# ryought/dbgphmm

Hardware: AMD Instinct MI355X
Metric: read-bases/sec through forward+backward P(R|X) (higher is better)
Workload: dtype f64; 1 GPU; cfg3: synthetic 100 kb diploid genome (1% divergence), 20x HiFi reads (p=0.001, L=1000), k=40 DBG; sparse-adaptive forward+backward+posteriors (generate_mappings); n_nodes=131694, n_edges=132357, reads_rank0=4026, bases_rank0=4000713, total_bases=4000713, spin_up_steps=12

## Files before the change

dbgphmm_amd/csrc/api.cpp:

```cpp
#include <chrono>
#include <cstdlib>
#include <cmath>
#include <cstring>

#include "phmm_internal.h"

namespace phmm {

static thread_local std::string g_error;
static thread_local hipStream_t g_stream = nullptr;
static thread_local uint64_t g_ws_limit = 0;
static thread_local CallStats g_stats;
static thread_local bool g_timing = false;

void set_error(const std::string &msg) { g_error = msg; }
int fail(int code, const std::string &msg) {
    g_error = msg;
    return code;
}
hipStream_t current_stream() { return g_stream; }
int &workset_index() {
    static thread_local int idx = 0;
    return idx;
}
// ... 50 lines not shown
    if (k.wide_bwd_t != 128 && k.wide_bwd_t != 448) k.wide_bwd_t = 0;
    k.wide_hinted_cpb = num("PHMM_WIDE_HINTED_CPB", 0);
    if (k.wide_hinted_cpb != 1 && k.wide_hinted_cpb != 2 && k.wide_hinted_cpb != 4) k.wide_hinted_cpb = 0;
    k.no_side_worker = flag("PHMM_NO_SIDE_WORKER");
    k.no_wide_handover = flag("PHMM_NO_WIDE_HANDOVER");
    k.workers = std::max(1, std::min(MAX_WORKERS, num("PHMM_WORKERS", 1)));
    k.warm_cols = num("PHMM_WARM_COLS", 0);
    k.chunk_groups = std::max(0, num("PHMM_CHUNK_GROUPS", 0));
    k.no_keep_all = flag("PHMM_NO_KEEP_ALL");
    k.pipeline_min_groups = std::max(1, num("PHMM_PIPELINE_MIN_GROUPS", 8));
    k.no_runmax = flag("PHMM_NO_RUNMAX");
    k.force_radix = flag("PHMM_FORCE_RADIX");
    k.no_bwd_skip = flag("PHMM_NO_BWD_SKIP");
    k.serial_emit = flag("PHMM_SERIAL_EMIT");
    k.emit_high_priority = flag("PHMM_EMIT_HIGH_PRIORITY");
    k.no_dma = flag("PHMM_NO_DMA");
    k.bwd_dma = flag("PHMM_BWD_DMA");
    k.dense_streams = num("PHMM_DENSE_STREAMS", 0);
    k.dense_w = num("PHMM_DENSE_W", 0);
    k.dense_npt = num("PHMM_DENSE_NPT", 0);
    if (const char *e = std::getenv("PHMM_MEM_FRACTION")) k.mem_fraction = std::min(0.97, std::max(0.1, std::atof(e)));
    k.share_prefix = num("PHMM_SHARE_PREFIX", -1);
    if (k.share_prefix < 0 || k.share_prefix > 6) k.share_prefix = -1;
    g_knobs = k;
}

void trace(const char *tag) {
    if (!g_knobs.trace) return;
    static thread_local std::chrono::steady_clock::time_point last = std::chrono::steady_clock::now();
    (void)hipStreamSynchronize(g_stream);
    const auto now = std::chrono::steady_clock::now();
    static const auto t0 = std::chrono::steady_clock::now();
    std::fprintf(stderr, "[phmm trace] w%d @%9.2f %-28s %8.2f ms\n", workset_index(),
                 std::chrono::duration<double, std::milli>(now - t0).count(), tag,
                 std::chrono::duration<double, std::milli>(now - last).count());
    last = now;
}

uint64_t table_budget(const DevicePool &pool, uint64_t reserve) {
    if (g_ws_limit) return g_ws_limit;
    size_t fr = 0, tot = 0;
    if (hipMemGetInfo(&fr, &tot) != hipSuccess) return (uint64_t)16 << 30;
    const double frac = g_knobs.mem_fraction > 0.0 ? g_knobs.mem_fraction : 0.9;
    const double b = frac * (double)(fr + pool.owned_table_bytes()) - (double)reserve;
    return (uint64_t)std::max(b, 64.0 * 1024 * 1024);
}
// ... 60 lines not shown
}
void flush_spare_buffers() { device_pool().flush_spares(); }

void DevicePool::release() {
    flush_spares();
    for (auto &w : wsets) w.release();
    ws_out.release();
    for (auto &ws : wstream)
        if (ws) {
            (void)hipStreamDestroy(ws);
            ws = nullptr;
        }
    for (auto &ws : cstream)
        if (ws) {
            (void)hipStreamDestroy(ws);
            ws = nullptr;
        }
    for (auto &we : cevent)
        for (auto &e : we)
            if (e) {
                (void)hipEventDestroy(e);
                e = nullptr;
            }
}

void copy_out(void *dst, const void *src_dev, size_t bytes) {
    if (!dst || !bytes) return;
    hipPointerAttribute_t at;
    const bool dev = hipPointerGetAttributes(&at, dst) == hipSuccess && at.type == hipMemoryTypeDevice;
    if (!dev) (void)hipGetLastError();
    HIP_CHECK(hipMemcpyAsync(dst, src_dev, bytes, dev ? hipMemcpyDeviceToDevice : hipMemcpyDeviceToHost,
                             current_stream()));
    HIP_CHECK(hipStreamSynchronize(current_stream()));
}

void put_bytes(void *dst, const void *src, size_t n) {
    if (!dst || !n) return;
    hipPointerAttribute_t at;
    if (hipPointerGetAttributes(&at, dst) == hipSuccess && at.type == hipMemoryTypeDevice) {
        HIP_CHECK(hipMemcpyAsync(dst, src, n, hipMemcpyHostToDevice, current_stream()));
        HIP_CHECK(hipStreamSynchronize(current_stream()));
    } else {
        (void)hipGetLastError();
        std::memcpy(dst, src, n);
    }
}
// ... 867 lines not shown
```

dbgphmm_amd/csrc/dense.hip:

```cpp
#include <algorithm>
#include <cmath>
#include <cstring>
#include <numeric>
#include <type_traits>

#include "dense_internal.h"
#include "lds_dma.h"
#include "prefix_share.h"

#ifndef PHMM_FWD_PF
#define PHMM_FWD_PF 2
#endif
#ifndef PHMM_BWD_PF
#define PHMM_BWD_PF 1
#endif
#ifndef PHMM_SMALLW_WAVES
#define PHMM_SMALLW_WAVES 3
#endif

namespace phmm {


__device__ __forceinline__ int xcd_block(int b, int nblk8) {
    int per = nblk8 >> 3;
// ... 66 lines not shown
        v += ror(v, std::integral_constant<int, 0x128>());
        v += ror(v, std::integral_constant<int, 0x124>());
        v += ror(v, std::integral_constant<int, 0x122>());
        v += ror(v, std::integral_constant<int, 0x121>());
        return v;
    }
#pragma unroll
    for (int off = 1; off < W; off <<= 1) v += __shfl_xor(v, off);
    return v;
}

struct OpMax {
    __device__ double operator()(double a, double b) const { return a > b ? a : b; }
};
struct OpAdd {
    __device__ double operator()(double a, double b) const { return a + b; }
};

template <int W, bool DMA>
__global__ void __launch_bounds__(BLOCK, (W == 64 ? 4 : PHMM_SMALLW_WAVES)) fwd_step(const DenseArgs a, const int pos) {
    __shared__ double lds[(BLOCK / 64) * 64];
    constexpr bool DMA_ = DMA && W == 64;
    __shared__ double ring[DMA_ ? (BLOCK / 64) * DMA_DEPTH * 128 : 1];
    const int g = blockIdx.y + a.g_off;
    const int lb = xcd_block(blockIdx.x, a.nblk8);
    constexpr int ROWS = BLOCK / W;
    const int r = threadIdx.x % W;
    const int row = threadIdx.x / W;
    const int len = a.len[g * W + r];
    const bool active = a.wf_sw == nullptr || a.wf_sw[g * W + r] < 0;
    const bool newcol = active && pos < len;
    const bool have_prev = active && pos >= 1 && pos <= len;
    const bool fin = have_prev && pos == len;
    if (!__syncthreads_or(newcol || have_prev)) return;
    const LinParams &lp = a.lp;
    const size_t NW = (size_t)a.N * W;

    int Epos = 0;
    double sc = 1.0, isc = 1.0, ibs = 0.0;
    double thrL = INFINITY, thrU = INFINITY;
    bool collect = false;
    if (have_prev) {
        const unsigned long long cm = a.cmaxF[((size_t)g * a.Lc + (pos - 1)) * W + r];
        const int Eprev = a.FE[((size_t)g * (a.Lc + 1) + (pos - 1)) * W + r];
        const double ib_st = exp(a.logib[pos - 1] - (double)Eprev * LN2);
        const unsigned long long ibb = (unsigned long long)__double_as_longlong(ib_st);
// ... 1397 lines not shown
```

dbgphmm_amd/csrc/dense_internal.h:

```cpp
#pragma once

#include <vector>

#include "phmm_internal.h"
#include "seg_hull.h"

namespace phmm {

static constexpr double LN2 = 0.693147180559945309417232121458;
static constexpr int BLOCK = 256;

struct DenseArgs {
    int N, ng, Lc, nblk, npt;
    int g_off;
    const NodeRec *nodes;
    const uint8_t *emis;
    const double *init, *dinit, *tdinit;
    const uint32_t *fc_off;
    const FwdEntry *fc;
    const uint32_t *bc_off;
    const BwdEntry *bc;
    const uint32_t *fh_off, *bh_off;
    const HopEntry *fh, *bh;
    int hop_mode;
    LinParams lp;
    const double *logib;
    const uint8_t *bases;
// ... 8 lines not shown
    double *Bm, *Bi, *Bd;
    int bcols;
    int *BE;
    unsigned long long *cmaxB;
    double *bpart;
    double *logmbB, *logibB;
    double *accg;
    int want_freq;
    int nblk8;
    unsigned long long *tmaxF;
    const int *bstart;
    int want_map;
    double *Pa, *Pb;
    double *Prun;
    unsigned long long *pmax;
    const int *wf_sw;
    const uint8_t *wf_mode;
    int *wf_sub;
    int *wf_cnt;
    uint32_t *wf_node;
    double *wf_tot;
    double wf_ratio;
    double wf_ub_a, wf_ub_b;
    const uint32_t *rs_off = nullptr, *rs = nullptr;
    uint32_t *skH = nullptr;
    uint8_t *skA = nullptr;
    int nrun = 0, nseg = 0, sseg = 1;
    unsigned long long *skcells = nullptr;
    const double *vFm = nullptr, *vFi = nullptr, *vFd = nullptr;
    const uint32_t *vlane = nullptr;
    int vLc = 0, vJ = 0;
};
static constexpr int WF_CAP = 1024;


struct Plan {
    int W, ng_total, npt, nblk, nblk8;
    std::vector<uint32_t> order;
};

Plan make_plan(const phmm_model *m, const phmm_reads *reads, int forced_w);
Plan make_plan_ids(const phmm_model *m, const phmm_reads *reads, const std::vector<uint32_t> &ids);
void layout(DenseArgs &a, int W, bool full_b, void *tables, void *misc, size_t &tb, size_t &mb,
            bool backward_only = false);
void fill_model_args(DenseArgs &a, const phmm_model *m);
void host_logib(const phmm_model *m, size_t n, std::vector<double> &out);
// ... 17 lines not shown
```

dbgphmm_amd/csrc/mapping_flow.hip:

```cpp
#include <algorithm>
#include <cmath>
#include <cstring>
#include <memory>

#include <hipcub/hipcub.hpp>

#include "sparse_dyn.h"
#include "lean_bwd_kernel.h"
#include "wide_bwd_kernel.h"

namespace phmm {

static constexpr int KMAX = PHMM_MAX_ACTIVE_NODES;

template <int CAP> struct FRec {
    double m[CAP], i[CAP], d[CAP];
    uint32_t id[CAP];
    int n, na, E;
};

template <int CAP> __device__ bool load_record(const RecPool &p, uint64_t pos_index, FRec<CAP> &f) {
    const uint64_t o1 = p.off[pos_index];
    if (o1 == 0) return false;
    const uint8_t *rec = p.base + (o1 - 8);
// ... 1151 lines not shown
                hipLaunchKernelGGL(emit_dense_small, dim3((unsigned)std::min(1024, (ub + BLOCK / 64 - 1) / (BLOCK / 64))), dim3(BLOCK), 0,
                                   s2, ma, pos, lanes);
                hipLaunchKernelGGL(emit_dense_map, dim3((unsigned)ub), dim3(BLOCK), 0, s2, ma, pos, lanes);
            }
            HIP_CHECK(hipEventRecord(ev_emit[par], s2));
            emitted[par] = true;
            if (st_on) st.launches[1]++;
        }
        for (int par = 0; par < 2; par++)
            if (emitted[par]) HIP_CHECK(hipStreamWaitEvent(s, ev_emit[par], 0));
        HIP_CHECK(hipGetLastError());
        const bool want_lb = mc.logb_out && pos_max >= 0 && lanes > 0;
        if (want_lb) {
            launch_bwd_finish(W, a);
            hipLaunchKernelGGL(gather_logb, dim3((unsigned)((lanes + BLOCK - 1) / BLOCK)), dim3(BLOCK), 0, s, (const double *)a.logmbB,
                               a.Lc, W, lanes, (double *)(cp + o_lb));
            HIP_CHECK(hipGetLastError());
        }
        st.ms[1] += lt.total_ms();
        for (int gi = 0; gi < lanes; gi++)
            if (st_on && !a.skcells && hb[gi] >= 0) st.cells[1] += (uint64_t)((hb[gi] & ~(1 << 30)) + 1) * m->N;
        const size_t err_words = (o_cells + sizeof(unsigned long long) - o_err) / sizeof(uint32_t);
        std::vector<uint32_t> herr(err_words);
        HIP_CHECK(hipMemcpyAsync(herr.data(), cp + o_err, sizeof(uint32_t) * err_words, hipMemcpyDeviceToHost, s));
        if (want_lb) HIP_CHECK(hipMemcpyAsync(mc.logb_out, cp + o_lb, sizeof(double) * lanes, hipMemcpyDeviceToHost, s));
        HIP_CHECK(hipStreamSynchronize(s));
        if (a.skcells) {
            unsigned long long nc = 0;
            memcpy(&nc, herr.data() + (o_cells - o_err) / sizeof(uint32_t), sizeof nc);
            st.cells[1] += nc;
        }
        if (dense_lock.owns_lock()) dense_lock.unlock();
        trace("  dense backward+collect");
        bool pool_full = false;
        for (int gi = 0; gi < lanes; gi++) {
            if (herr[gi] & SP_ERR_POOL) pool_full = true;
            else if (herr[gi] & ~SP_STOP_SLICE) PHMM_THROW(PHMM_EINTERNAL, "mapping backward error " + std::to_string(herr[gi]));
        }
        if (!pool_full) break;
        (void)attempt;
        throw SinkOverflow{};
    }
}

__global__ void __launch_bounds__(BLOCK) map_counts(RecPool mp, uint64_t n_pos, uint64_t *cnt) {
    const uint64_t p = (uint64_t)blockIdx.x * BLOCK + threadIdx.x;
    if (p > n_pos) return;
    uint64_t c = 0;
    if (p < n_pos) {
// ... 91 lines not shown
static void finish_mappings(phmm_model *m, const phmm_reads *reads, MappingSink &sink, const std::vector<double> &lf,
                            const std::vector<double> &lb, phmm_mappings **out, double *out_node_freq) {
    hipStream_t s = current_stream();
    const uint64_t n_pos = reads->total;
    std::unique_ptr<phmm_mappings> mp(new phmm_mappings());
    mp->R = reads->R;
    mp->total_pos = n_pos;
    mp->read_off = reads->off;
    mp->read_logp = lf;
    mp->read_logp_backward = lb;
    mp->host_valid = false;
    mp->trusted = true;
    (void)hipGetDevice(&mp->device);
    DevicePool &dpool = device_pool();
    DevBuf &cnt = m->wset().aux[13], &tmp = m->wset().aux[14];
    cnt.reserve(sizeof(uint64_t) * (n_pos + 1));
    dpool.take(mp->d_pos_off, sizeof(uint64_t) * (n_pos + 1));
    const unsigned nb = (unsigned)((n_pos + 1 + BLOCK - 1) / BLOCK);
    hipLaunchKernelGGL(map_counts, dim3(nb), dim3(BLOCK), 0, s, sink.mp, n_pos, cnt.as<uint64_t>());
    size_t tb = 0;
    HIP_CHECK(hipcub::DeviceScan::ExclusiveSum(nullptr, tb, cnt.as<uint64_t>(), mp->d_pos_off.as<uint64_t>(), (int)(n_pos + 1), s));
    tmp.reserve(tb);
    HIP_CHECK(hipcub::DeviceScan::ExclusiveSum(tmp.p, tb, cnt.as<uint64_t>(), mp->d_pos_off.as<uint64_t>(), (int)(n_pos + 1), s));
    uint64_t total = 0;
    HIP_CHECK(hipMemcpyAsync(&total, mp->d_pos_off.as<uint64_t>() + n_pos, sizeof(uint64_t), hipMemcpyDeviceToHost, s));
    HIP_CHECK(hipStreamSynchronize(s));
    mp->total_entries = total;
    dpool.take(mp->d_nodes, sizeof(uint32_t) * std::max<uint64_t>(total, 1));
    dpool.take(mp->d_logp, sizeof(double) * std::max<uint64_t>(total, 1));
    hipLaunchKernelGGL(map_compact, dim3(nb), dim3(BLOCK), 0, s, sink.mp, n_pos, mp->d_pos_off.as<uint64_t>(),
                       mp->d_nodes.as<uint32_t>(), mp->d_logp.as<double>());
    DevBuf &d_roff = m->wset().aux[15], &d_rmax = m->wset().aux[16];
    d_roff.upload(reads->off.data(), sizeof(uint64_t) * (reads->R + 1));
    d_rmax.reserve(sizeof(uint32_t) * reads->R);
    hipLaunchKernelGGL(map_read_max, dim3((unsigned)((reads->R + BLOCK / 64 - 1) / (BLOCK / 64))), dim3(BLOCK), 0, s,
                       d_roff.as<uint64_t>(), reads->R, mp->d_pos_off.as<uint64_t>(), d_rmax.as<uint32_t>());
    mp->read_max_list.resize(reads->R);
    HIP_CHECK(hipMemcpyAsync(mp->read_max_list.data(), d_rmax.p, sizeof(uint32_t) * reads->R, hipMemcpyDeviceToHost, s));
    HIP_CHECK(hipStreamSynchronize(s));
    mp->on_device = true;
    trace("device CSR");
    if (out_node_freq) {
        DevBuf &d_prob = m->wset().aux[17], &d_sn = m->wset().aux[18], &d_sp = m->wset().aux[19], &d_freq = m->wset().aux[20];
        const uint64_t n = std::max<uint64_t>(total, 1);
        d_prob.reserve(sizeof(double) * n);
        d_sn.reserve(sizeof(uint32_t) * n);
        d_sp.reserve(sizeof(double) * n);
        d_freq.reserve(sizeof(double) * m->N);
        if (total) {
            hipLaunchKernelGGL(map_probs, dim3((unsigned)((total + BLOCK - 1) / BLOCK)), dim3(BLOCK), 0, s,
                               mp->d_logp.as<double>(), total, d_prob.as<double>());
            int end_bit = 1;
            while (end_bit < 32 && (1ull << end_bit) < m->N) end_bit++;
            size_t sb = 0;
            HIP_CHECK(hipcub::DeviceRadixSort::SortPairs(nullptr, sb, mp->d_nodes.as<uint32_t>(), d_sn.as<uint32_t>(),
                                                         d_prob.as<double>(), d_sp.as<double>(), (int)total, 0, end_bit, s));
            tmp.reserve(sb);
            HIP_CHECK(hipcub::DeviceRadixSort::SortPairs(tmp.p, sb, mp->d_nodes.as<uint32_t>(), d_sn.as<uint32_t>(),
                                                         d_prob.as<double>(), d_sp.as<double>(), (int)total, 0, end_bit, s));
        }
        hipLaunchKernelGGL(map_node_freq, dim3((m->N + NODE_FREQ_WAVES - 1) / NODE_FREQ_WAVES), dim3(64 * NODE_FREQ_WAVES), 0, s, d_sn.as<uint32_t>(),
// ... 659 lines not shown
```

dbgphmm_amd/csrc/phmm_internal.h:

```cpp
#pragma once

#include <hip/hip_runtime.h>

#include <cstdint>
#include <cstdio>
#include <memory>
#include <mutex>
#include <string>
#include <vector>

#include "../../include/phmm_amd.h"
#include "../../include/phmm_amd_states.h"
#include "../../include/phmm_amd_path.h"
#include "../../include/phmm_amd_share.h"
#include "../../include/phmm_amd_sample.h"
#include "../../include/phmm_amd_generate.h"
#include "../../include/phmm_amd_align.h"

namespace phmm {

void set_error(const std::string &msg);
int fail(int code, const std::string &msg);

struct Error {
    int code;
    std::string msg;
};
#define PHMM_THROW(code, msg) throw ::phmm::Error{(code), (msg)}
// ... 63 lines not shown
void copy_out(void *dst, const void *src_dev, size_t bytes);

struct WorkSet {
    DevBuf tables, misc, aux[24];
    size_t bytes() const {
        size_t b = tables.bytes + misc.bytes;
        for (const auto &a : aux) b += a.bytes;
        return b;
    }
    void release() {
        tables.release();
        misc.release();
        for (auto &a : aux) a.release();
    }
};
static constexpr int MAX_WORKERS = 4;
struct DevicePool {
    int device = 0;
    std::recursive_mutex call_mu;
    WorkSet wsets[MAX_WORKERS];
    hipStream_t wstream[MAX_WORKERS] = {};
    hipStream_t cstream[MAX_WORKERS] = {};
    hipEvent_t cevent[MAX_WORKERS][4] = {};
    DevBuf ws_out;
    static constexpr size_t SPARE_MAX = 6, SPARE_BYTES = (size_t)8 << 30;
    std::mutex spare_mu;
    std::vector<std::pair<void *, size_t>> spare;
    size_t spare_total = 0;
    void recycle(DevBuf &b);
    void take(DevBuf &b, size_t n);
    void flush_spares();
    size_t owned_table_bytes() const {
        size_t b = 0;
        for (const auto &w : wsets) b += w.tables.bytes;
        return b;
    }
    size_t owned_bytes() const {
        size_t b = ws_out.bytes + spare_total;
        for (const auto &w : wsets) b += w.bytes();
        return b;
    }
    void release();
};
DevicePool &device_pool();

struct LinParams {
    double p_mismatch, p_match, p_random, p_end;
    double p_MM, p_IM, p_DM, p_MI, p_II, p_DI, p_MD, p_ID, p_DD;
    int n_max_gaps;
};

struct FwdEntry {
    uint32_t node;
    uint32_t pad;
    double w1, wD, wT;
};
struct BwdEntry {
    uint32_t node;
    uint32_t emis;
    double c1, cAd, cAt, cQd;
};

struct HopEntry {
    uint32_t node;
    uint32_t hop_emis;
    double w;
};
// ... 152 lines not shown
CallStats &stats();
bool timing_enabled();
struct ShareInfo {
    int J = 0;
    uint64_t lanes = 0;
};
ShareInfo &share_info();

struct LaunchTimer {
    bool on;
    std::vector<hipEvent_t> ev;
    explicit LaunchTimer(bool on_) : on(on_) {}
    ~LaunchTimer() {
        for (auto e : ev) (void)hipEventDestroy(e);
    }
    void begin() {
        if (!on) return;
        hipEvent_t e;
        HIP_CHECK(hipEventCreate(&e));
        HIP_CHECK(hipEventRecord(e, current_stream()));
        ev.push_back(e);
    }
    void end() { begin(); }
    double total_ms() {
        if (!on || ev.empty()) return 0.0;
        HIP_CHECK(hipEventSynchronize(ev.back()));
        double t = 0.0;
        for (size_t k = 0; k + 1 < ev.size(); k += 2) {
            float ms = 0;
            HIP_CHECK(hipEventElapsedTime(&ms, ev[k], ev[k + 1]));
            t += ms;
        }
        return t;
    }
};

void trace(const char *tag);

struct Knobs {
    bool trace = false;
    bool no_lean = false;
    bool no_wide_class = false;
    bool no_packed = false;
    int packed_cpl = 0;
    bool no_exact_hinted = false;
    bool no_exact_dense = false;
// ... 3 lines not shown
    bool wide_edge_bwd = false;
    bool wide_states_bwd = false;
    int wide_bwd_t = 0;
    int wide_hinted_cpb = 0;
    bool no_side_worker = false;
    bool no_wide_handover = false;
    int workers = 1;
    int warm_cols = 0;
    int chunk_groups = 0;
    bool no_keep_all = false;
    int pipeline_min_groups = 8;
    bool no_runmax = false;
    bool force_radix = false;
    bool serial_emit = false;
    bool emit_high_priority = false;
    bool no_dma = false;
    bool bwd_dma = false;
    bool no_bwd_skip = false;
    int dense_streams = 0;
    int dense_w = 0;
    int dense_npt = 0;
    double mem_fraction = 0.0;
    int share_prefix = -1;
};
const Knobs &knobs();
void refresh_knobs();

void model_build_host(phmm_model *m);
void model_upload(phmm_model *m);
const RunSucc &model_run_successors(phmm_model *m, int seg);

void run_dense(phmm_model *m, const phmm_reads *reads, double *out_lf, double *out_lb,
               double *out_nf);
void full_prob_sparse_backward(phmm_model *m, const phmm_reads *reads, double *out_logp, double *out_total);
void backward_sparse_tables(phmm_model *m, const uint8_t *read, uint64_t len, double *b_m, double *b_i, double *b_d,
                            double *b_scal, uint8_t *is_dense);
void run_sparse(phmm_model *m, const phmm_reads *reads, double *out_lf, double *out_lb, double *out_nf);
void run_dense_edges(phmm_model *m, const phmm_reads *reads, double *out_lf, double *out_ef, double *out_if);
struct RecPool;
void full_prob_reads_hinted(phmm_model *m, const phmm_reads *reads, const phmm_mappings *mp, uint32_t n_cand,
                            const double *init_logp, const double *trans_logp, double *out_logp,
                            double *out_total, const RecPool *pool = nullptr, const uint32_t *copy_nums = nullptr,
                            uint32_t min_copy_num = 0);
void full_prob_reads_copy_num_changes(phmm_model *m, const phmm_reads *reads, const phmm_mappings *mp,
                                      const uint32_t *base_cn, uint32_t min_cn, uint32_t n_cand, const uint64_t *chg_off,
                                      const uint32_t *chg_node, const uint32_t *chg_cn, double *out_logp,
// ... 50 lines not shown
```

dbgphmm_amd/csrc/sparse_dyn.hip:

```cpp
#include <algorithm>
#include <cmath>
#include <cstdlib>
#include <cstring>

#include "dense_internal.h"
#include <condition_variable>
#include <deque>
#include <exception>
#include <functional>
#include <memory>
#include <mutex>
#include <thread>

#include "frontier_dev.h"
#include "prefix_share.h"
#include "sparse_dyn.h"
#include "sparse_fwd_kernel.h"
#include "wide_fwd_kernel.h"
#include "lean_fwd_kernel.h"

namespace phmm {

struct WarmArgs {
    DenseArgs d;
    int *sw;
    int *cnt;
    uint32_t *cand_node;
    double *cand_tot;
    int *cand_n;
    int *undecided;
    int *amb;
    int *n_amb;
    double ratio_lin;
    int n_warmup, threshold;
};

struct StageArgs {
    const uint8_t *bases;
    const uint64_t *off;
    const uint32_t *order;
    uint32_t n_slots;
    int W, Lc, Lfull;
    uint8_t *out_dense, *out_full;
};
__global__ void __launch_bounds__(BLOCK) stage_bases(const StageArgs sa) {
    const int g = blockIdx.y;
    const unsigned t = blockIdx.x * BLOCK + threadIdx.x;
    if (t >= (unsigned)sa.Lfull * sa.W) return;
    const int i = (int)(t / sa.W), r = (int)(t % sa.W);
    const uint32_t slot = (uint32_t)g * sa.W + r;
    uint8_t b = 0xff;
    if (slot < sa.n_slots) {
        const uint32_t rd = sa.order[slot];
        const uint64_t o0 = sa.off[rd], o1 = sa.off[rd + 1];
        if ((uint64_t)i < o1 - o0) b = sa.bases[o0 + i];
    }
    sa.out_full[((size_t)g * sa.Lfull + i) * sa.W + r] = b;
// ... 60 lines not shown
    }
    if (wa.sw[gi] >= 0 || !wa.amb[gi]) return;
    bool decided = false;
    if (pos >= len) {
        wa.sw[gi] = len;
        decided = true;
    } else if (pos >= 1) {
        const int c = wa.cnt[gi];
        const int ntop = c < PHMM_MAX_ACTIVE_NODES ? c : PHMM_MAX_ACTIVE_NODES;
        if (pos >= wa.n_warmup || ntop <= wa.threshold) {
            wa.sw[gi] = pos;
            wa.cand_n[gi] = c;
            decided = true;
        }
    }
    if (!decided) atomicAdd(wa.undecided, 1);
    wa.cnt[gi] = 0;
}

__global__ void __launch_bounds__(BLOCK) warm_decide_fused(const WarmArgs wa, const int pos, const int total_lanes, const int W) {
    const int gi = blockIdx.x * (BLOCK / 64) + (threadIdx.x >> 6);
    const int lane = threadIdx.x & 63;
    if (gi >= total_lanes) return;
    const int len = wa.d.len[gi];
    if (len == 0) {
        if (lane == 0) wa.sw[gi] = 0;
        return;
    }
    if (wa.sw[gi] >= 0) return;
    const int nsub = wa.d.wf_sub[gi], cn = wa.d.wf_cnt[gi];
    const bool collected = wa.d.wf_mode[gi] != 0 && cn <= WF_CAP;
    bool decided = false, amb = false;
    int new_sw = -1, new_cn = 0;
    if (pos >= len) {
        new_sw = len;
        decided = true;
    } else if (pos >= 1) {
        const bool forced = pos >= wa.n_warmup;
        if (collected) {
            const int g = gi / W, r = gi % W;
            const double tmax = __longlong_as_double((long long)wa.d.tmaxF[((size_t)g * wa.d.Lc + (pos - 1)) * W + r]);
            const double thr = tmax * wa.ratio_lin;
            int c = 0;
            for (int base = 0; base < cn; base += 64) {
                const int j = base + lane;
                const double t = j < cn ? wa.d.wf_tot[(size_t)gi * WF_CAP + j] : 0.0;
                const bool ok = j < cn && t > 0.0 && t > thr;
                const unsigned long long mask = __ballot(ok);
                const int slot = c + __popcll(mask & ((1ull << lane) - 1ull));
                if (ok && slot < PHMM_MAX_ACTIVE_NODES) {
                    wa.cand_node[(size_t)gi * PHMM_MAX_ACTIVE_NODES + slot] = wa.d.wf_node[(size_t)gi * WF_CAP + j];
                    wa.cand_tot[(size_t)gi * PHMM_MAX_ACTIVE_NODES + slot] = t;
                }
                c += __popcll(mask);
// ... 386 lines not shown
        base.nblk8 = plan.nblk8;
        base.npt = plan.npt;
        base.eall = 0;
        base.want_freq = 0;
        {
        DenseArgs a = base;
        a.ng = ngc;
        a.Lc = Lc;
        size_t tb = 0, mb = 0;
        layout(a, W, false, nullptr, nullptr, tb, mb);
        m->wset().tables.reserve(tb);
        m->wset().misc.reserve(mb);
        layout(a, W, false, m->wset().tables.p, m->wset().misc.p, tb, mb);
        HIP_CHECK(hipMemsetAsync(m->wset().misc.p, 0, mb, s));
        const int lanes = ngc * W;
        size_t wb = 0;
        auto carve = [&](size_t bytes) {
            wb = (wb + 255) / 256 * 256;
            size_t o = wb;
            wb += bytes;
            return o;
        };
        const size_t o_sw = carve(sizeof(int) * lanes), o_cnt = carve(sizeof(int) * lanes),
                     o_cn = carve(sizeof(int) * lanes), o_und = carve(sizeof(int) * 2),
                     o_amb = carve(sizeof(int) * lanes), o_wsub = carve(sizeof(int) * lanes),
                     o_wcnt = carve(sizeof(int) * lanes), o_mode = carve((size_t)lanes),
                     o_cnode = carve(sizeof(uint32_t) * (size_t)lanes * PHMM_MAX_ACTIVE_NODES),
                     o_ctot = carve(sizeof(double) * (size_t)lanes * PHMM_MAX_ACTIVE_NODES),
                     o_lanes = carve(sizeof(uint32_t) * lanes), o_out = carve(sizeof(double) * lanes),
                     o_err = carve(sizeof(uint32_t) * lanes),
                     o_wnode = carve(sizeof(uint32_t) * (size_t)lanes * WF_CAP),
                     o_wtot = carve(sizeof(double) * (size_t)lanes * WF_CAP),
                     o_bases = carve((size_t)ngc * Lfull * W);
        const bool shared = share.J > 0 && it.pc->may_defer && by_ratio && W == SHARE_W;
        const size_t o_vlane = carve(shared ? sizeof(uint32_t) * lanes : 0);
        warm.reserve(wb);
        char *wp = (char *)warm.p;
        HIP_CHECK(hipMemsetAsync(wp, 0, o_cnode, s));
        HIP_CHECK(hipMemsetAsync(wp + o_sw, 0xff, sizeof(int) * lanes, s));

        trace("chunk setup");
        if (knobs().trace)
            std::fprintf(stderr, "      chunk: groups %d..%d of %d, W %d, kept columns %d, longest read %d\n", g0, g0 + ngc, plan.ng_total, W, Lc, Lfull);
        std::vector<int> hl((size_t)lanes, 0);
        uint64_t dense_cells = 0;
        for (int gi = 0; gi < lanes; gi++) {
            const size_t slot = (size_t)g0 * W + gi;
// ... 76 lines not shown
        if (shared) {
            ShareArgs sa{share.va, a, a.vlane, share.J};
            const int nrange = (int)((m->N + SHARE_ROWS - 1) / SHARE_ROWS), nrange8 = (nrange + 7) / 8 * 8;
            lt.begin();
            hipLaunchKernelGGL(share_copy_ctl, dim3((lanes + BLOCK - 1) / BLOCK), dim3(BLOCK), 0, s, sa, lanes);
            hipLaunchKernelGGL(share_expand, dim3((unsigned)nrange8 * (unsigned)ngc), dim3(BLOCK), 0, s, sa, nrange);
            lt.end();
            HIP_CHECK(hipGetLastError());
            pos = share.J;
        }
        if (!by_ratio) {
            const int last = std::min<int>((int)prm.n_warmup, Lc);
            for (pos = 0; pos <= last; pos++) {
                lt.begin();
                launch_fwd_step(W, a, pos);
                lt.end();
                if (st_on) st.launches[0]++;
            }
            std::vector<int> fsw(lanes);
            for (int gi = 0; gi < lanes; gi++) fsw[gi] = std::min<int>((int)prm.n_warmup, hl[gi]);
            HIP_CHECK(hipMemcpyAsync(wa.sw, fsw.data(), sizeof(int) * lanes, hipMemcpyHostToDevice, s));
            HIP_CHECK(hipStreamSynchronize(s));
        }
        for (; by_ratio; pos++) {
            lt.begin();
            launch_fwd_step(W, a, pos);
            lt.end();
            if (st_on) st.launches[0]++;
            HIP_CHECK(hipMemsetAsync(wa.undecided, 0, sizeof(int) * 2, s));
            hipLaunchKernelGGL(warm_decide_fused, dim3((lanes + BLOCK / 64 - 1) / (BLOCK / 64)), dim3(BLOCK), 0, s, wa, pos,
                               lanes, W);
            int und[2] = {0, 0};
            HIP_CHECK(hipMemcpyAsync(und, wa.undecided, sizeof(int) * 2, hipMemcpyDeviceToHost, s));
            HIP_CHECK(hipStreamSynchronize(s));
            if (und[1] > 0) {
                launch_col_count_w(W, wa, pos - 1);
                hipLaunchKernelGGL(warm_decide, dim3((lanes + BLOCK - 1) / BLOCK), dim3(BLOCK), 0, s, wa, pos, lanes);
                HIP_CHECK(hipMemcpyAsync(und, wa.undecided, sizeof(int), hipMemcpyDeviceToHost, s));
                HIP_CHECK(hipStreamSynchronize(s));
                st.launches[3]++;
            }
            if (und[0] == 0) break;
            if (pos >= Lc) PHMM_THROW(PHMM_EINTERNAL, "warm-up did not terminate");
        }
        st.ms[0] += lt.total_ms();
        if (dense_lock.owns_lock()) dense_lock.unlock();
        trace("dense warm-up");
        launch_fwd_finish(W, a);
        std::vector<int> hsw(lanes);
        std::vector<int> hcn(lanes);
        std::vector<double> tlf(lanes);
        std::vector<double> tlb(lanes, 0.0);
        HIP_CHECK(hipMemcpyAsync(hsw.data(), wa.sw, sizeof(int) * lanes, hipMemcpyDeviceToHost, s));
        HIP_CHECK(hipMemcpyAsync(hcn.data(), wa.cand_n, sizeof(int) * lanes, hipMemcpyDeviceToHost, s));
        HIP_CHECK(hipMemcpyAsync(tlf.data(), a.logPf, sizeof(double) * lanes, hipMemcpyDeviceToHost, s));
        HIP_CHECK(hipStreamSynchronize(s));
        {
            for (int gi = 0; gi < lanes; gi++)
                if (hl[gi] > Lc && hsw[gi] >= Lc) {
                    if (!deferred) PHMM_THROW(PHMM_EINTERNAL, "warm-up ran past n_warmup");
                    const size_t slot = (size_t)g0 * W + gi;
                    deferred->push_back(plan.order[slot]);
                    new_flags[plan.order[slot]] |= PHMM_READ_DEFERRED;
                    if (knobs().trace)
                        std::fprintf(stderr, "      read %u (len %d) still dense at column %d: deferred\n", plan.order[slot],
                                     hl[gi], Lc);
// ... 109 lines not shown
                fa.lane_pos0 = d_lp0;
                std::vector<uint32_t> todo = sparse_lanes;
                std::vector<uint32_t> herr(lanes);
                std::vector<int> hstop(lanes);
                bool pool_full = false;
                const bool lean_ok =
                    by_ratio && m->dev.max_degree <= (uint32_t)ADJ_DEG && !knobs().no_lean;
                const bool wide_ok = lean_ok && !knobs().no_wide_class;
                auto run_phase = [&](int phase, int steps, const std::vector<uint32_t> &who, std::vector<uint32_t> &rest,
                                     std::vector<uint32_t> &wide) {
                    rest.clear();
                    wide.clear();
                    auto launch = [&](int kind, int mode, const std::vector<uint32_t> &l) {
                        HIP_CHECK(hipMemcpyAsync(wp + o_lanes, l.data(), l.size() * sizeof(uint32_t), hipMemcpyHostToDevice, s));
                        fa.mode = mode;
                        fa.max_steps = steps;
                        const dim3 grid((unsigned)l.size());
                        if (kind == 0) hipLaunchKernelGGL(lean_forward_kernel, grid, dim3(64), 0, s, fa);
                        else if (kind == 1) hipLaunchKernelGGL(wide_forward_kernel, grid, dim3(WFK_T), 0, s, fa);
                        else if (kind == 3) hipLaunchKernelGGL((sparse_forward_kernel<128>), grid, dim3(64), 0, s, fa);
                        else hipLaunchKernelGGL((sparse_forward_kernel<PHMM_MAX_ACTIVE_NODES>), grid, dim3(64), 0, s, fa);
                        HIP_CHECK(hipGetLastError());
                        st.launches[2]++;
                        HIP_CHECK(hipMemcpyAsync(herr.data(), fa.err, sizeof(uint32_t) * lanes, hipMemcpyDeviceToHost, s));
                        HIP_CHECK(hipMemcpyAsync(hstop.data(), fa.stop, sizeof(int) * lanes, hipMemcpyDeviceToHost, s));
                        HIP_CHECK(hipStreamSynchronize(s));
                    };
                    if (phase == 1) launch(lean_ok ? 0 : 3, 1, who);
                    else launch(wide_ok ? 1 : 2, phase == 0 ? 0 : 1, who);
                    for (uint32_t gi : who) {
                        if (herr[gi] & SP_ERR_POOL) pool_full = true;
                        else if ((herr[gi] & SP_ERR_CAPACITY) && phase != 1)
                            PHMM_THROW(PHMM_ECAPACITY, "sparse forward: frontier does not fit 400 slots");
                        else if (herr[gi] & ~SP_ERR_CAPACITY)
                            PHMM_THROW(PHMM_EINTERNAL, "sparse forward error " + std::to_string(herr[gi]));
                        if (hstop[gi] < hl[gi]) ((phase == 1 && (herr[gi] & SP_ERR_CAPACITY)) ? wide : rest).push_back(gi);
                    }
                    trace(phase == 0 ? "   phase A <400>" : (phase == 1 ? "   phase B <64>" : "   phase C <400>"));
                    if (knobs().trace) std::fprintf(stderr, "      remaining lanes %zu (+ %zu wide)\n", rest.size(), wide.size());
                };
                const bool can_hand_over = deferred && by_ratio && single_mode && side_on && !knobs().no_wide_handover;
                const int b_slice = (can_hand_over && Lfull > 3072) ? 2048 : 0;
                size_t handed = 0;
                int bursts = 0;
                std::vector<uint32_t> rest, wide, tmp1, tmp2;
                run_phase(0, 6, todo, rest, wide);
                todo.swap(rest);
                for (int turn = 0; turn < 100000 && !todo.empty() && !pool_full; turn++) {
                    run_phase(1, b_slice, todo, rest, wide);
// ... 242 lines not shown
    }
    const int n_threads = (int)std::min<size_t>((size_t)n_workers, queue.size());
    if (!short_ids.empty()) {
        std::unique_ptr<PlanCtx> pc(new PlanCtx{make_plan_ids(m, reads, short_ids), (int64_t)prm.n_warmup + 2, false, {}});
        const size_t side_group = ((size_t)(prm.n_warmup + 2) * 24 + 4 * 8 + (size_t)map_planes * 8) * m->N * pc->plan.W;
        std::lock_guard<std::mutex> lk(mu);
        if (n_threads <= 1 && side_on && side_group <= limit_side) {
            enqueue_plan(std::move(pc), side_queue);
            side_started = true;
            start_side_worker();
        } else {
            enqueue_plan(std::move(pc), queue);
        }
    }
    if (n_threads <= 1) {
        single_mode = true;
        worker_loop();
        {
            std::lock_guard<std::mutex> lk(mu);
            main_done = true;
        }
        cv.notify_all();
        if (side_started && side_thread.joinable()) {
            side_thread.join();
            CallStats &st = stats();
            for (int k = 0; k < 5; k++) {
                st.ms[k] += side_stats.ms[k];
                st.launches[k] += side_stats.launches[k];
                st.cells[k] += side_stats.cells[k];
            }
        }
    } else {
        HIP_CHECK(hipStreamSynchronize(current_stream()));
        const ThreadContext ctx = capture_thread_context();
        CallStats merged;
        for (int t = 0; t < n_threads; t++)
            if (!m->pool->wstream[t]) HIP_CHECK(hipStreamCreateWithFlags(&m->pool->wstream[t], hipStreamNonBlocking));
        std::vector<std::thread> threads;
        struct JoinAll {
            std::vector<std::thread> &t;
            ~JoinAll() {
                for (auto &th : t)
                    if (th.joinable()) th.join();
            }
        } join_all{threads};
        threads.reserve(n_threads);
        for (int t = 0; t < n_threads; t++) {
// ... 36 lines not shown
```

Before: 36.56 million bases/s.

## Speculatively issue next warm-up column with device-side gate and pinned staging

The warm-up loop now enqueues column pos+1 before waiting on column pos. A device-side gate read from the previous column's undecided/ambiguous counters makes the kernels exit early if the speculation was wrong. This removes one host round-trip of latency per warm-up column. Small device-to-host readbacks (error flags, stop positions, CSR totals) now go through a per-worker pinned staging buffer, and the CSR total readback is merged with the read-max copy. The cost is extra gated kernel launches that may do nothing, added complexity in the double-buffered counter slots, and a fallback exact-count path that still synchronizes.

New measurement: 36.80 million bases/s (median of 6 runs). No clear change (+0.7%).

```diff
diff --git a/dbgphmm_amd/csrc/api.cpp b/dbgphmm_amd/csrc/api.cpp
--- a/dbgphmm_amd/csrc/api.cpp
+++ b/dbgphmm_amd/csrc/api.cpp
@@ -96,6 +96,9 @@
     if (const char *e = std::getenv("PHMM_MEM_FRACTION")) k.mem_fraction = std::min(0.97, std::max(0.1, std::atof(e)));
     k.share_prefix = num("PHMM_SHARE_PREFIX", -1);
     if (k.share_prefix < 0 || k.share_prefix > 6) k.share_prefix = -1;
+    k.trace_join = flag("PHMM_TRACE_JOIN");
+    k.no_warm_ahead = flag("PHMM_NO_WARM_AHEAD");
+    k.no_fused_count = flag("PHMM_NO_FUSED_COUNT");
     g_knobs = k;
 }
 
@@ -202,6 +205,26 @@
                 (void)hipEventDestroy(e);
                 e = nullptr;
             }
+    for (auto &we : wevent)
+        for (auto &e : we)
+            if (e) {
+                (void)hipEventDestroy(e);
+                e = nullptr;
+            }
+    for (auto &p : pinned)
+        if (p) {
+            (void)hipHostFree(p);
+            p = nullptr;
+        }
+}
+
+void *DevicePool::pinned_block(int worker) {
+    if (!pinned[worker]) HIP_CHECK(hipHostMalloc(&pinned[worker], PINNED_BYTES, hipHostMallocDefault));
+    return pinned[worker];
+}
+hipEvent_t DevicePool::warm_event(int worker, int slot) {
+    if (!wevent[worker][slot]) HIP_CHECK(hipEventCreateWithFlags(&wevent[worker][slot], hipEventDisableTiming));
+    return wevent[worker][slot];
 }
 
 void copy_out(void *dst, const void *src_dev, size_t bytes) {
diff --git a/dbgphmm_amd/csrc/dense.hip b/dbgphmm_amd/csrc/dense.hip
--- a/dbgphmm_amd/csrc/dense.hip
+++ b/dbgphmm_amd/csrc/dense.hip
@@ -112,6 +112,7 @@
     __shared__ double lds[(BLOCK / 64) * 64];
     constexpr bool DMA_ = DMA && W == 64;
     __shared__ double ring[DMA_ ? (BLOCK / 64) * DMA_DEPTH * 128 : 1];
+    if (a.wf_gate != nullptr && warm_gate_closed(a.wf_gate[0], a.wf_gate[1])) return;
     const int g = blockIdx.y + a.g_off;
     const int lb = xcd_block(blockIdx.x, a.nblk8);
     constexpr int ROWS = BLOCK / W;
diff --git a/dbgphmm_amd/csrc/dense_internal.h b/dbgphmm_amd/csrc/dense_internal.h
--- a/dbgphmm_amd/csrc/dense_internal.h
+++ b/dbgphmm_amd/csrc/dense_internal.h
@@ -3,6 +3,7 @@
 #include <vector>
 
 #include "phmm_internal.h"
+#include "warm_ahead.h"
 #include "seg_hull.h"
 
 namespace phmm {
@@ -57,6 +58,7 @@
     double *wf_tot;
     double wf_ratio;
     double wf_ub_a, wf_ub_b;
+    const int *wf_gate = nullptr;
     const uint32_t *rs_off = nullptr, *rs = nullptr;
     uint32_t *skH = nullptr;
     uint8_t *skA = nullptr;
diff --git a/dbgphmm_amd/csrc/mapping_flow.hip b/dbgphmm_amd/csrc/mapping_flow.hip
--- a/dbgphmm_amd/csrc/mapping_flow.hip
+++ b/dbgphmm_amd/csrc/mapping_flow.hip
@@ -1197,9 +1197,10 @@
             if (st_on && !a.skcells && hb[gi] >= 0) st.cells[1] += (uint64_t)((hb[gi] & ~(1 << 30)) + 1) * m->N;
         const size_t err_words = (o_cells + sizeof(unsigned long long) - o_err) / sizeof(uint32_t);
         std::vector<uint32_t> herr(err_words);
-        HIP_CHECK(hipMemcpyAsync(herr.data(), cp + o_err, sizeof(uint32_t) * err_words, hipMemcpyDeviceToHost, s));
-        if (want_lb) HIP_CHECK(hipMemcpyAsync(mc.logb_out, cp + o_lb, sizeof(double) * lanes, hipMemcpyDeviceToHost, s));
-        HIP_CHECK(hipStreamSynchronize(s));
+        PinnedStage pin(*m->pool);
+        pin.fetch(herr.data(), cp + o_err, sizeof(uint32_t) * err_words, s);
+        if (want_lb) pin.fetch(mc.logb_out, cp + o_lb, sizeof(double) * lanes, s);
+        pin.sync(s);
         if (a.skcells) {
             unsigned long long nc = 0;
             memcpy(&nc, herr.data() + (o_cells - o_err) / sizeof(uint32_t), sizeof nc);
@@ -1337,21 +1338,22 @@
     HIP_CHECK(hipcub::DeviceScan::ExclusiveSum(nullptr, tb, cnt.as<uint64_t>(), mp->d_pos_off.as<uint64_t>(), (int)(n_pos + 1), s));
     tmp.reserve(tb);
     HIP_CHECK(hipcub::DeviceScan::ExclusiveSum(tmp.p, tb, cnt.as<uint64_t>(), mp->d_pos_off.as<uint64_t>(), (int)(n_pos + 1), s));
-    uint64_t total = 0;
-    HIP_CHECK(hipMemcpyAsync(&total, mp->d_pos_off.as<uint64_t>() + n_pos, sizeof(uint64_t), hipMemcpyDeviceToHost, s));
-    HIP_CHECK(hipStreamSynchronize(s));
-    mp->total_entries = total;
-    dpool.take(mp->d_nodes, sizeof(uint32_t) * std::max<uint64_t>(total, 1));
-    dpool.take(mp->d_logp, sizeof(double) * std::max<uint64_t>(total, 1));
-    hipLaunchKernelGGL(map_compact, dim3(nb), dim3(BLOCK), 0, s, sink.mp, n_pos, mp->d_pos_off.as<uint64_t>(),
-                       mp->d_nodes.as<uint32_t>(), mp->d_logp.as<double>());
     DevBuf &d_roff = m->wset().aux[15], &d_rmax = m->wset().aux[16];
     d_roff.upload(reads->off.data(), sizeof(uint64_t) * (reads->R + 1));
     d_rmax.reserve(sizeof(uint32_t) * reads->R);
     hipLaunchKernelGGL(map_read_max, dim3((unsigned)((reads->R + BLOCK / 64 - 1) / (BLOCK / 64))), dim3(BLOCK), 0, s,
                        d_roff.as<uint64_t>(), reads->R, mp->d_pos_off.as<uint64_t>(), d_rmax.as<uint32_t>());
     mp->read_max_list.resize(reads->R);
-    HIP_CHECK(hipMemcpyAsync(mp->read_max_list.data(), d_rmax.p, sizeof(uint32_t) * reads->R, hipMemcpyDeviceToHost, s));
+    uint64_t total = 0;
+    PinnedStage pin(dpool);
+    pin.fetch(&total, mp->d_pos_off.as<uint64_t>() + n_pos, sizeof(uint64_t), s);
+    pin.fetch(mp->read_max_list.data(), d_rmax.p, sizeof(uint32_t) * reads->R, s);
+    pin.sync(s);
+    mp->total_entries = total;
+    dpool.take(mp->d_nodes, sizeof(uint32_t) * std::max<uint64_t>(total, 1));
+    dpool.take(mp->d_logp, sizeof(double) * std::max<uint64_t>(total, 1));
+    hipLaunchKernelGGL(map_compact, dim3(nb), dim3(BLOCK), 0, s, sink.mp, n_pos, mp->d_pos_off.as<uint64_t>(),
+                       mp->d_nodes.as<uint32_t>(), mp->d_logp.as<double>());
     HIP_CHECK(hipStreamSynchronize(s));
     mp->on_device = true;
     trace("device CSR");
diff --git a/dbgphmm_amd/csrc/phmm_internal.h b/dbgphmm_amd/csrc/phmm_internal.h
--- a/dbgphmm_amd/csrc/phmm_internal.h
+++ b/dbgphmm_amd/csrc/phmm_internal.h
@@ -4,6 +4,7 @@
 
 #include <cstdint>
 #include <cstdio>
+#include <cstring>
 #include <memory>
 #include <mutex>
 #include <string>
@@ -113,6 +114,11 @@
     hipStream_t wstream[MAX_WORKERS] = {};
     hipStream_t cstream[MAX_WORKERS] = {};
     hipEvent_t cevent[MAX_WORKERS][4] = {};
+    static constexpr size_t PINNED_BYTES = (size_t)256 << 10;
+    void *pinned[MAX_WORKERS] = {};
+    hipEvent_t wevent[MAX_WORKERS][2] = {};
+    void *pinned_block(int worker);
+    hipEvent_t warm_event(int worker, int slot);
     DevBuf ws_out;
     static constexpr size_t SPARE_MAX = 6, SPARE_BYTES = (size_t)8 << 30;
     std::mutex spare_mu;
@@ -134,6 +140,35 @@
     void release();
 };
 DevicePool &device_pool();
+
+struct PinnedStage {
+    static constexpr size_t PINNED_RESERVED = 64;
+    struct Pending {
+        void *dst;
+        const char *src;
+        size_t n;
+    };
+    char *base;
+    size_t used = PINNED_RESERVED;
+    std::vector<Pending> pending;
+    explicit PinnedStage(DevicePool &pool) : base((char *)pool.pinned_block(workset_index())) {}
+    void fetch(void *dst, const void *dev, size_t n, hipStream_t s) {
+        const size_t o = (used + 63) / 64 * 64;
+        if (o + n <= DevicePool::PINNED_BYTES) {
+            HIP_CHECK(hipMemcpyAsync(base + o, dev, n, hipMemcpyDeviceToHost, s));
+            pending.push_back(Pending{dst, base + o, n});
+            used = o + n;
+        } else {
+            HIP_CHECK(hipMemcpyAsync(dst, dev, n, hipMemcpyDeviceToHost, s));
+        }
+    }
+    void sync(hipStream_t s) {
+        HIP_CHECK(hipStreamSynchronize(s));
+        for (const Pending &p : pending) std::memcpy(p.dst, p.src, p.n);
+        pending.clear();
+        used = PINNED_RESERVED;
+    }
+};
 
 struct LinParams {
     double p_mismatch, p_match, p_random, p_end;
@@ -332,6 +367,13 @@
         ev.push_back(e);
     }
     void end() { begin(); }
+    void drop_last() {
+        if (!on || ev.size() < 2) return;
+        for (int k = 0; k < 2; k++) {
+            (void)hipEventDestroy(ev.back());
+            ev.pop_back();
+        }
+    }
     double total_ms() {
         if (!on || ev.empty()) return 0.0;
         HIP_CHECK(hipEventSynchronize(ev.back()));
@@ -381,6 +423,9 @@
     int dense_npt = 0;
     double mem_fraction = 0.0;
     int share_prefix = -1;
+    bool trace_join = false;
+    bool no_warm_ahead = false;
+    bool no_fused_count = false;
 };
 const Knobs &knobs();
 void refresh_knobs();
diff --git a/dbgphmm_amd/csrc/sparse_dyn.hip b/dbgphmm_amd/csrc/sparse_dyn.hip
--- a/dbgphmm_amd/csrc/sparse_dyn.hip
+++ b/dbgphmm_amd/csrc/sparse_dyn.hip
@@ -1,4 +1,5 @@
 #include <algorithm>
+#include <chrono>
 #include <cmath>
 #include <cstdlib>
 #include <cstring>
@@ -33,6 +34,8 @@
     int *n_amb;
     double ratio_lin;
     int n_warmup, threshold;
+    const int *gate;
+    int no_fused;
 };
 
 struct StageArgs {
@@ -139,6 +142,7 @@
     const int gi = blockIdx.x * (BLOCK / 64) + (threadIdx.x >> 6);
     const int lane = threadIdx.x & 63;
     if (gi >= total_lanes) return;
+    if (wa.gate != nullptr && warm_gate_closed(wa.gate[0], wa.gate[1])) return;
     const int len = wa.d.len[gi];
     if (len == 0) {
         if (lane == 0) wa.sw[gi] = 0;
@@ -146,7 +150,7 @@
     }
     if (wa.sw[gi] >= 0) return;
     const int nsub = wa.d.wf_sub[gi], cn = wa.d.wf_cnt[gi];
-    const bool collected = wa.d.wf_mode[gi] != 0 && cn <= WF_CAP;
+    const bool collected = wa.d.wf_mode[gi] != 0 && cn <= WF_CAP && !wa.no_fused;
     bool decided = false, amb = false;
     int new_sw = -1, new_cn = 0;
     if (pos >= len) {
@@ -579,7 +583,7 @@
             return o;
         };
         const size_t o_sw = carve(sizeof(int) * lanes), o_cnt = carve(sizeof(int) * lanes),
-                     o_cn = carve(sizeof(int) * lanes), o_und = carve(sizeof(int) * 2),
+                     o_cn = carve(sizeof(int) * lanes), o_und = carve(sizeof(int) * WARM_SLOTS * WARM_SLOT_INTS),
                      o_amb = carve(sizeof(int) * lanes), o_wsub = carve(sizeof(int) * lanes),
                      o_wcnt = carve(sizeof(int) * lanes), o_mode = carve((size_t)lanes),
                      o_cnode = carve(sizeof(uint32_t) * (size_t)lanes * PHMM_MAX_ACTIVE_NODES),
@@ -702,26 +706,56 @@
             HIP_CHECK(hipMemcpyAsync(wa.sw, fsw.data(), sizeof(int) * lanes, hipMemcpyHostToDevice, s));
             HIP_CHECK(hipStreamSynchronize(s));
         }
+        int *const und_dev = (int *)(wp + o_und);
+        volatile int *const und_host = (volatile int *)m->pool->pinned_block(workset_index());
+        const bool ahead_on = by_ratio && !knobs().no_warm_ahead;
+        wa.no_fused = knobs().no_fused_count ? 1 : 0;
+        auto issue_column = [&](int p, bool gated) {
+            const int so = warm_slot_offset(p);
+            const int *gate = gated ? und_dev + warm_slot_offset(p - 1) : nullptr;
+            DenseArgs ag = a;
+            ag.wf_gate = gate;
+            wa.undecided = und_dev + so;
+            wa.n_amb = wa.undecided + 1;
+            wa.gate = gate;
+            lt.begin();
+            launch_fwd_step(W, ag, p);
+            lt.end();
+            HIP_CHECK(hipMemsetAsync(wa.undecided, 0, sizeof(int) * WARM_SLOT_INTS, s));
+            hipLaunchKernelGGL(warm_decide_fused, dim3((lanes + BLOCK / 64 - 1) / (BLOCK / 64)), dim3(BLOCK), 0, s, wa, p,
+                               lanes, W);
+            HIP_CHECK(hipMemcpyAsync((void *)(und_host + so), wa.undecided, sizeof(int) * WARM_SLOT_INTS, hipMemcpyDeviceToHost, s));
+            HIP_CHECK(hipEventRecord(m->pool->warm_event(workset_index(), warm_slot(p)), s));
+        };
+        if (by_ratio) {
+            issue_column(pos, false);
+            if (st_on) st.launches[0]++;
+        }
         for (; by_ratio; pos++) {
-            lt.begin();
-            launch_fwd_step(W, a, pos);
-            lt.end();
-            if (st_on) st.launches[0]++;
-            HIP_CHECK(hipMemsetAsync(wa.undecided, 0, sizeof(int) * 2, s));
-            hipLaunchKernelGGL(warm_decide_fused, dim3((lanes + BLOCK / 64 - 1) / (BLOCK / 64)), dim3(BLOCK), 0, s, wa, pos,
-                               lanes, W);
-            int und[2] = {0, 0};
-            HIP_CHECK(hipMemcpyAsync(und, wa.undecided, sizeof(int) * 2, hipMemcpyDeviceToHost, s));
-            HIP_CHECK(hipStreamSynchronize(s));
-            if (und[1] > 0) {
+            const bool went_ahead = warm_may_go_ahead(ahead_on, pos, Lc);
+            if (went_ahead) issue_column(pos + 1, true);
+            const int so = warm_slot_offset(pos);
+            HIP_CHECK(hipEventSynchronize(m->pool->warm_event(workset_index(), warm_slot(pos))));
+            const int undecided = und_host[so], n_amb = und_host[so + 1];
+            int undecided_final = undecided;
+            const bool ahead_ran = warm_ahead_ran(went_ahead, undecided, n_amb);
+            if (went_ahead && !ahead_ran) lt.drop_last();
+            if (warm_needs_exact(n_amb)) {
+                wa.undecided = und_dev + so;
+                wa.n_amb = wa.undecided + 1;
+                wa.gate = nullptr;
                 launch_col_count_w(W, wa, pos - 1);
                 hipLaunchKernelGGL(warm_decide, dim3((lanes + BLOCK - 1) / BLOCK), dim3(BLOCK), 0, s, wa, pos, lanes);
-                HIP_CHECK(hipMemcpyAsync(und, wa.undecided, sizeof(int), hipMemcpyDeviceToHost, s));
+                HIP_CHECK(hipMemcpyAsync((void *)(und_host + so), wa.undecided, sizeof(int), hipMemcpyDeviceToHost, s));
                 HIP_CHECK(hipStreamSynchronize(s));
+                undecided_final = und_host[so];
                 st.launches[3]++;
             }
-            if (und[0] == 0) break;
+            const bool finished = warm_finished(undecided_final);
+            if (finished) break;
             if (pos >= Lc) PHMM_THROW(PHMM_EINTERNAL, "warm-up did not terminate");
+            if (warm_reissue(finished, ahead_ran)) issue_column(pos + 1, false);
+            if (st_on) st.launches[0]++;
         }
         st.ms[0] += lt.total_ms();
         if (dense_lock.owns_lock()) dense_lock.unlock();
@@ -877,9 +911,10 @@
                         else hipLaunchKernelGGL((sparse_forward_kernel<PHMM_MAX_ACTIVE_NODES>), grid, dim3(64), 0, s, fa);
                         HIP_CHECK(hipGetLastError());
                         st.launches[2]++;
-                        HIP_CHECK(hipMemcpyAsync(herr.data(), fa.err, sizeof(uint32_t) * lanes, hipMemcpyDeviceToHost, s));
-                        HIP_CHECK(hipMemcpyAsync(hstop.data(), fa.stop, sizeof(int) * lanes, hipMemcpyDeviceToHost, s));
-                        HIP_CHECK(hipStreamSynchronize(s));
+                        PinnedStage pin(*m->pool);
+                        pin.fetch(herr.data(), fa.err, sizeof(uint32_t) * lanes, s);
+                        pin.fetch(hstop.data(), fa.stop, sizeof(int) * lanes, s);
+                        pin.sync(s);
                     };
                     if (phase == 1) launch(lean_ok ? 0 : 3, 1, who);
                     else launch(wide_ok ? 1 : 2, phase == 0 ? 0 : 1, who);
@@ -1168,7 +1203,11 @@
         }
         cv.notify_all();
         if (side_started && side_thread.joinable()) {
+            const auto j0 = std::chrono::steady_clock::now();
             side_thread.join();
+            if (knobs().trace || knobs().trace_join)
+                std::fprintf(stderr, "[phmm trace] w%d join: waited %.3f ms for the side plans\n", workset_index(),
+                             std::chrono::duration<double, std::milli>(std::chrono::steady_clock::now() - j0).count());
             CallStats &st = stats();
             for (int k = 0; k < 5; k++) {
                 st.ms[k] += side_stats.ms[k];
diff --git a/dbgphmm_amd/csrc/warm_ahead.h b/dbgphmm_amd/csrc/warm_ahead.h
--- /dev/null
+++ b/dbgphmm_amd/csrc/warm_ahead.h
@@ -0,0 +1,26 @@
+#pragma once
+
+#if defined(__HIPCC__)
+#define PHMM_WARM_FN __host__ __device__ inline
+#else
+#define PHMM_WARM_FN inline
+#endif
+
+namespace phmm {
+
+static constexpr int WARM_SLOTS = 2, WARM_SLOT_INTS = 2;
+PHMM_WARM_FN int warm_slot(int pos) { return pos & (WARM_SLOTS - 1); }
+PHMM_WARM_FN int warm_slot_offset(int pos) { return warm_slot(pos) * WARM_SLOT_INTS; }
+
+PHMM_WARM_FN bool warm_may_go_ahead(bool enabled, int pos, int Lc) { return enabled && pos + 1 <= Lc; }
+
+PHMM_WARM_FN bool warm_gate_closed(int undecided, int n_amb) { return n_amb > 0 || undecided == 0; }
+
+PHMM_WARM_FN bool warm_needs_exact(int n_amb) { return n_amb > 0; }
+PHMM_WARM_FN bool warm_ahead_ran(bool went_ahead, int undecided, int n_amb) {
+    return went_ahead && !warm_gate_closed(undecided, n_amb);
+}
+PHMM_WARM_FN bool warm_finished(int undecided_final) { return undecided_final == 0; }
+PHMM_WARM_FN bool warm_reissue(bool finished, bool ahead_ran) { return !finished && !ahead_ran; }
+
+}
```
